# idcrook/tweeker_raytracer

Measured on NVIDIA B200. Metric: rtigo3_geometry_1080p_samples_per_s, higher is better.
Workload: dtype f32

## Files before the change

### tweeker_raytracer_b200/csrc/trace.cuh

```cuda
#pragma once

#include "rtc_internal.h"

#ifndef RTC_I2F_AXES
#define RTC_I2F_AXES 1
#endif
#ifndef RTC_RESTORE_WORLD
#define RTC_RESTORE_WORLD 1
#endif
#ifndef RTC_TRI_MINMAX
#define RTC_TRI_MINMAX 1
#endif
#ifndef RTC_LEAF_THRESHOLD
#define RTC_LEAF_THRESHOLD 0
#endif
#ifndef RTC_ONE_TRI_PER_STEP
#define RTC_ONE_TRI_PER_STEP 0
#endif
#ifndef RTC_FETCH_THRESHOLD
#define RTC_FETCH_THRESHOLD 12
#endif
#ifndef RTC_TRACE_MIN_BLOCKS
#define RTC_TRACE_MIN_BLOCKS 8
#endif

struct TraceHit
{
  float    t, u, v;
  uint32_t inst, prim;
};

struct ObjRay
{
  float dx, dy, dz;
  float Sx, Sy, Sz;
  int   kx, ky, kz;
};

__device__ __forceinline__ float sel3(float x, float y, float z, int k)
{
#if defined(__CUDACC__)
  float r;
  asm("{\n\t.reg .pred p1, p2;\n\tsetp.eq.s32 p1, %4, 1;\n\tsetp.eq.s32 p2, %4, 2;\n\tselp.f32 %0, %2, %1, p1;\n\tselp.f32 %0, %3, %0, p2;\n\t}"
      : "=&f"(r) : "f"(x), "f"(y), "f"(z), "r"(k));
  return r;
#else
  return (k == 2) ? z : ((k == 1) ? y : x);
#endif
}

__device__ __forceinline__ void shear_setup(ObjRay& r)
{
  const float ax = fabsf(r.dx), ay = fabsf(r.dy), az = fabsf(r.dz);
  int kz = (ax >= ay && ax >= az) ? 0 : ((ay >= az) ? 1 : 2);
  int kx = kz + 1; if (kx == 3) kx = 0;
  int ky = kx + 1; if (ky == 3) ky = 0;
  const float dz = sel3(r.dx, r.dy, r.dz, kz);
  if (dz < 0.0f) { const int t = kx; kx = ky; ky = t; }
  r.kx = kx; r.ky = ky; r.kz = kz;
  r.Sx = __fdiv_rn(sel3(r.dx, r.dy, r.dz, kx), dz);
  r.Sy = __fdiv_rn(sel3(r.dx, r.dy, r.dz, ky), dz);
  r.Sz = __fdiv_rn(1.0f, dz);
}

__device__ __forceinline__ float pick3(float x, float y, float z, bool is1, bool is2)
{
  float r = is1 ? y : x;
  return is2 ? z : r;
}

__device__ __forceinline__ bool tri_test(const ObjRay& r, float ox, float oy, float oz, const float4 v0, const float4 v1, const float4 v2,
                                         float& t, float& det, float& V, float& W)
{
  const float A0 = __fsub_rn(v0.x, ox), A1 = __fsub_rn(v0.y, oy), A2 = __fsub_rn(v0.z, oz);
  const float B0 = __fsub_rn(v1.x, ox), B1 = __fsub_rn(v1.y, oy), B2 = __fsub_rn(v1.z, oz);
  const float C0 = __fsub_rn(v2.x, ox), C1 = __fsub_rn(v2.y, oy), C2 = __fsub_rn(v2.z, oz);
  const bool x1 = r.kx == 1, x2 = r.kx == 2, y1 = r.ky == 1, y2 = r.ky == 2, z1 = r.kz == 1, z2 = r.kz == 2;
  const float Akz = pick3(A0, A1, A2, z1, z2), Bkz = pick3(B0, B1, B2, z1, z2), Ckz = pick3(C0, C1, C2, z1, z2);
  const float Ax = __fmaf_rn(-r.Sx, Akz, pick3(A0, A1, A2, x1, x2)), Ay = __fmaf_rn(-r.Sy, Akz, pick3(A0, A1, A2, y1, y2));
  const float Bx = __fmaf_rn(-r.Sx, Bkz, pick3(B0, B1, B2, x1, x2)), By = __fmaf_rn(-r.Sy, Bkz, pick3(B0, B1, B2, y1, y2));
  const float Cx = __fmaf_rn(-r.Sx, Ckz, pick3(C0, C1, C2, x1, x2)), Cy = __fmaf_rn(-r.Sy, Ckz, pick3(C0, C1, C2, y1, y2));
  float U = __fsub_rn(__fmul_rn(Cx, By), __fmul_rn(Cy, Bx));
  V = __fsub_rn(__fmul_rn(Ax, Cy), __fmul_rn(Ay, Cx));
  W = __fsub_rn(__fmul_rn(Bx, Ay), __fmul_rn(By, Ax));
  if (U == 0.0f || V == 0.0f || W == 0.0f)
  {
    U = (float)__dsub_rn(__dmul_rn((double)Cx, (double)By), __dmul_rn((double)Cy, (double)Bx));
    V = (float)__dsub_rn(__dmul_rn((double)Ax, (double)Cy), __dmul_rn((double)Ay, (double)Cx));
    W = (float)__dsub_rn(__dmul_rn((double)Bx, (double)Ay), __dmul_rn((double)By, (double)Ax));
  }
#if RTC_TRI_MINMAX
  if (fminf(fminf(U, V), W) < 0.0f && fmaxf(fmaxf(U, V), W) > 0.0f) return false;
#else
  if ((U < 0.0f || V < 0.0f || W < 0.0f) && (U > 0.0f || V > 0.0f || W > 0.0f)) return false;
#endif
  det = __fadd_rn(__fadd_rn(U, V), W);
  if (det == 0.0f) return false;
  const float Az = __fmul_rn(r.Sz, Akz), Bz = __fmul_rn(r.Sz, Bkz), Cz = __fmul_rn(r.Sz, Ckz);
  const float T = __fmaf_rn(U, Az, __fmaf_rn(V, Bz, __fmul_rn(W, Cz)));
  t = __fdiv_rn(T, det);
  return true;
}

struct BoxRay
{
  float idx, idy, idz;
  float ox, oy, oz;
  uint32_t octinv;
};

template <bool EXACT>
__device__ __forceinline__ float fast_rcp(float d)
{
  if (fabsf(d) < 0x1p-80f) d = copysignf(0x1p-80f, d);
  if (EXACT) return __frcp_rn(d);
#if defined(__CUDACC__)
  float r;
  asm("rcp.approx.ftz.f32 %0, %1;" : "=f"(r) : "f"(d));
  return r;
#else
  return 1.0f / d;
#endif
}

template <bool EXACT = false>
__device__ __forceinline__ void box_setup(BoxRay& b, float ox, float oy, float oz, float dx, float dy, float dz)
{
  b.idx = fast_rcp<EXACT>(dx); b.idy = fast_rcp<EXACT>(dy); b.idz = fast_rcp<EXACT>(dz);
  b.ox = ox; b.oy = oy; b.oz = oz;
  const uint32_t oct = ((dx < 0.0f) ? 4u : 0u) | ((dy < 0.0f) ? 2u : 0u) | ((dz < 0.0f) ? 1u : 0u);
  b.octinv = 7u ^ oct;
}

template <uint32_t I>
__device__ __forceinline__ float quant_f(uint32_t w, uint32_t bias)
{
#if defined(__CUDACC__)
  uint32_t r;
  asm("prmt.b32 %0, %1, %2, %3;" : "=r"(r) : "r"(w), "r"(bias), "n"(0x7404u | (I << 4)));
  return __uint_as_float(r);
#else
  return __uint_as_float((bias & 0xff000000u) | ((bias & 0xffu) << 16) | (((w >> (8u * I)) & 0xffu) << 8) | (bias & 0xffu));
#endif
}

template <uint32_t I>
__device__ __forceinline__ float quant_i2f(uint32_t w)
{
  return (float)((w >> (8u * I)) & 0xffu);
}

__device__ __forceinline__ float sat_idir(float id, uint32_t eb)
{
  const uint32_t raw = 0xB7000000u - (eb << 23);
  const float lim = __uint_as_float(raw < 0x7F000000u ? raw : 0x7F000000u);
  return fminf(fmaxf(id, -lim), lim);
}

__device__ __forceinline__ uint32_t node_test(const BoxRay& b, const uint4 n0, const uint4 n2, const uint4 n3, const uint4 n4,
                                              float tmin, float tlimit, uint32_t opaqueZero)
{
  const uint32_t e = n0.w;
  const float idx = sat_idir(b.idx, e & 0xffu), idy = sat_idir(b.idy, (e >> 8) & 0xffu), idz = sat_idir(b.idz, (e >> 16) & 0xffu);
  const float adjx = __uint_as_float((e & 0xffu) << 23) * idx;
  const float adjy = __uint_as_float(((e >> 8) & 0xffu) << 23) * idy;
  const float adjz = __uint_as_float(((e >> 16) & 0xffu) << 23) * idz;
  const float orgx = fmaf(-32768.0f, adjx, (__uint_as_float(n0.x) - b.ox) * idx);
#if RTC_I2F_AXES >= 2
  const float orgy = (__uint_as_float(n0.y) - b.oy) * idy;
#else
  const float orgy = fmaf(-32768.0f, adjy, (__uint_as_float(n0.y) - b.oy) * idy);
#endif
#if RTC_I2F_AXES >= 1
  const float orgz = (__uint_as_float(n0.z) - b.oz) * idz;
#else
  const float orgz = fmaf(-32768.0f, adjz, (__uint_as_float(n0.z) - b.oz) * idz);
#endif
  const bool nx = b.idx < 0.0f, ny = b.idy < 0.0f, nz = b.idz < 0.0f;
  const uint32_t nearx[2] = { nx ? n3.z : n2.x, nx ? n3.w : n2.y }, farx[2] = { nx ? n2.x : n3.z, nx ? n2.y : n3.w };
  const uint32_t neary[2] = { ny ? n4.x : n2.z, ny ? n4.y : n2.w }, fary[2] = { ny ? n2.z : n4.x, ny ? n2.w : n4.y };
  const uint32_t nearz[2] = { nz ? n4.z : n3.x, nz ? n4.w : n3.y }, farz[2] = { nz ? n3.x : n4.z, nz ? n3.y : n4.w };
  const float tlimitPad = tlimit * (1.0f + 0x1p-17f);
  const uint32_t bias = 0x47000000u + opaqueZero;
  uint32_t hits = 0;
#if RTC_I2F_AXES >= 1
#define RTC_QZ(I, W) quant_i2f<I>(W)
#else
#define RTC_QZ(I, W) quant_f<I>(W, bias)
#endif
#if RTC_I2F_AXES >= 2
#define RTC_QY(I, W) quant_i2f<I>(W)
#else
#define RTC_QY(I, W) quant_f<I>(W, bias)
#endif
#define RTC_BOX(S, H, I) \
  { \
    const float t0x = fmaf(quant_f<I>(nearx[H], bias), adjx, orgx), t1x = fmaf(quant_f<I>(farx[H], bias), adjx, orgx); \
    const float t0y = fmaf(RTC_QY(I, neary[H]), adjy, orgy), t1y = fmaf(RTC_QY(I, fary[H]), adjy, orgy); \
    const float t0z = fmaf(RTC_QZ(I, nearz[H]), adjz, orgz), t1z = fmaf(RTC_QZ(I, farz[H]), adjz, orgz); \
    const float tn = fmaxf(fmaxf(fmaxf(t0x, t0y), t0z), tmin); \
    const float tf = fminf(fminf(fminf(t1x, t1y), t1z) * (1.0f + 0x1p-17f), tlimitPad); \
    if (tn <= tf) hits |= 1u << S; \
  }
  RTC_BOX(0, 0, 0) RTC_BOX(1, 0, 1) RTC_BOX(2, 0, 2) RTC_BOX(3, 0, 3)
  RTC_BOX(4, 1, 0) RTC_BOX(5, 1, 1) RTC_BOX(6, 1, 2) RTC_BOX(7, 1, 3)
#undef RTC_BOX
#undef RTC_QZ
#undef RTC_QY
  return hits;
}

__device__ __forceinline__ uint32_t xor_permute8(uint32_t h, uint32_t x)
{
  if (x & 1u) h = ((h & 0xAAu) >> 1) | ((h & 0x55u) << 1);
  if (x & 2u) h = ((h & 0xCCu) >> 2) | ((h & 0x33u) << 2);
  if (x & 4u) h = ((h & 0xF0u) >> 4) | ((h & 0x0Fu) << 4);
  return h;
}

struct TraceCounts { uint32_t nodes, tris, insts; };

#define RTC_SM_STACK 8
#if RTC_RESTORE_WORLD
#define RTC_SM_RAY_WORDS 15
#else
#define RTC_SM_RAY_WORDS 11
#endif
#define RTC_LM_STACK 32

#ifndef RTC_STACK_OVERFLOW_COUNTER
#define RTC_STACK_OVERFLOW_COUNTER g_rtcStackOverflows
#endif
__device__ unsigned int RTC_STACK_OVERFLOW_COUNTER = 0;

template <bool ANY, bool COUNT, int BLOCK, bool SKIP = false, int TRICAP = RTC_ONE_TRI_PER_STEP>
struct Traversal
{
  float skipT; uint32_t skipInst, skipPrim;
  float* smRay;
  float tmin, tlimit;
  float hitT;
  uint32_t hitInst, hitPrim;
  uint2 nodeGroup, triGroup;
  int sp, blasBase;
  uint32_t curInst;
  BoxRay br;
  ObjRay orr;
  const uint4*  nodes;
  uint2* smStack;
  uint2* lmStack;
  TraceCounts counts;

  __device__ __forceinline__ void push(uint2 v)
  {
    if (sp < RTC_SM_STACK) smStack[sp * BLOCK] = v;
    else if (sp < RTC_SM_STACK + RTC_LM_STACK) lmStack[sp - RTC_SM_STACK] = v;
    else { atomicAdd(&RTC_STACK_OVERFLOW_COUNTER, 1u); return; }
    ++sp;
  }
  __device__ __forceinline__ uint2 pop()
  {
    --sp;
    return (sp < RTC_SM_STACK) ? smStack[sp * BLOCK] : lmStack[(sp - RTC_SM_STACK) & (RTC_LM_STACK - 1)];
  }

  __device__ __forceinline__ bool found() const { return hitInst != 0xffffffffu; }

  __device__ __forceinline__ TraceHit result() const
  {
    TraceHit h;
    h.t = -1.0f; h.u = 0.0f; h.v = 0.0f; h.inst = 0xffffffffu; h.prim = 0xffffffffu;
    if (found())
    {
      h.t = hitT; h.inst = hitInst; h.prim = hitPrim;
      if (!ANY) { const float det = smRay[8 * BLOCK]; h.u = __fdiv_rn(smRay[6 * BLOCK], det); h.v = __fdiv_rn(smRay[7 * BLOCK], det); }
    }
    return h;
  }

  __device__ __forceinline__ bool begin(const SceneDesc& sc, const float4 o, const float4 d)
  {
    smRay[0] = o.x; smRay[BLOCK] = o.y; smRay[2 * BLOCK] = o.z;
    smRay[3 * BLOCK] = d.x; smRay[4 * BLOCK] = d.y; smRay[5 * BLOCK] = d.z;
    tmin = o.w; tlimit = d.w;
    hitT = -1.0f; hitInst = 0xffffffffu; hitPrim = 0xffffffffu;
    if (COUNT) { counts.nodes = 0; counts.tris = 0; counts.insts = 0; }
    if (!(tlimit > tmin)) return false;
    sp = 0; blasBase = -1; curInst = 0;
    box_setup<COUNT>(br, o.x, o.y, o.z, d.x, d.y, d.z);
#if RTC_RESTORE_WORLD
    smRay[11 * BLOCK] = br.idx; smRay[12 * BLOCK] = br.idy; smRay[13 * BLOCK] = br.idz; smRay[14 * BLOCK] = __uint_as_float(br.octinv);
#endif
    nodes = sc.tlasNodes;
    nodeGroup = make_uint2(0u, 0x80000000u);
    triGroup = make_uint2(0u, 0u);
    return true;
  }

  __device__ __forceinline__ bool has_leaves() const { return triGroup.y != 0u; }

  __device__ __forceinline__ void node_phase()
  {
    if (nodeGroup.y & 0xff000000u)
    {
      const uint32_t bit = 31u - (uint32_t)__clz((int)nodeGroup.y);
      nodeGroup.y &= ~(1u << bit);
      if (nodeGroup.y & 0xff000000u) push(nodeGroup);
      const uint32_t slot = (bit - 24u) ^ br.octinv;
      const uint32_t rel = (uint32_t)__popc(nodeGroup.y & 0xffu & ((1u << slot) - 1u));
      const uint4* np = nodes + (size_t)(nodeGroup.x + rel) * 5u;
      const uint4 n0 = __ldg(np), n1 = __ldg(np + 1), n2 = __ldg(np + 2), n3 = __ldg(np + 3), n4 = __ldg(np + 4);
      if (COUNT) counts.nodes++;
      const uint32_t hits = node_test(br, n0, n2, n3, n4, tmin, tlimit, n1.x >> 31);
      const uint32_t imask = n0.w >> 24;
      nodeGroup = make_uint2(n1.x, (xor_permute8(hits & imask, br.octinv) << 24) | imask);
      uint32_t leaf = hits & ~imask, primMask = 0u;
      while (leaf)
      {
        const uint32_t s = (uint32_t)__ffs((int)leaf) - 1u;
        leaf &= leaf - 1u;
        const uint32_t meta = (((s < 4u) ? n1.z : n1.w) >> (8u * (s & 3u))) & 0xffu;
        primMask |= ((1u << (meta >> 5)) - 1u) << (meta & 31u);
      }
      triGroup = make_uint2(n1.y, primMask);
    }
    else
    {
      triGroup = nodeGroup;
      nodeGroup = make_uint2(0u, 0u);
    }
  }

  __device__ __forceinline__ bool leaf_phase(const SceneDesc& sc)
  {
    int tested = 0;
    while (triGroup.y)
    {
      const uint32_t idx = (uint32_t)__ffs((int)triGroup.y) - 1u;
      triGroup.y &= triGroup.y - 1u;
      if (blasBase < 0)
      {
        const uint32_t inst = __ldg(sc.tlasLeaves + triGroup.x + idx);
        if (triGroup.y) push(triGroup);
        if (nodeGroup.y & 0xff000000u) push(nodeGroup);
        const float4* ip = sc.instances + (size_t)inst * 4u;
        const float4 r0 = __ldg(ip), r1 = __ldg(ip + 1), r2 = __ldg(ip + 2), r3 = __ldg(ip + 3);
        if (COUNT) counts.insts++;
        const float wox = smRay[0], woy = smRay[BLOCK], woz = smRay[2 * BLOCK];
        const float wdx = smRay[3 * BLOCK], wdy = smRay[4 * BLOCK], wdz = smRay[5 * BLOCK];
        const float oox = __fmaf_rn(r0.x, wox, __fmaf_rn(r0.y, woy, __fmaf_rn(r0.z, woz, r0.w)));
        const float ooy = __fmaf_rn(r1.x, wox, __fmaf_rn(r1.y, woy, __fmaf_rn(r1.z, woz, r1.w)));
        const float ooz = __fmaf_rn(r2.x, wox, __fmaf_rn(r2.y, woy, __fmaf_rn(r2.z, woz, r2.w)));
        orr.dx = __fmaf_rn(r0.x, wdx, __fmaf_rn(r0.y, wdy, __fmul_rn(r0.z, wdz)));
        orr.dy = __fmaf_rn(r1.x, wdx, __fmaf_rn(r1.y, wdy, __fmul_rn(r1.z, wdz)));
        orr.dz = __fmaf_rn(r2.x, wdx, __fmaf_rn(r2.y, wdy, __fmul_rn(r2.z, wdz)));
        shear_setup(orr);
        box_setup<COUNT>(br, oox, ooy, ooz, orr.dx, orr.dy, orr.dz);
        curInst = inst;
        blasBase = sp;
        nodes = reinterpret_cast<const uint4*>(((unsigned long long)__float_as_uint(r3.y) << 32) | __float_as_uint(r3.x));
        smRay[9 * BLOCK] = r3.z; smRay[10 * BLOCK] = r3.w;
        nodeGroup = make_uint2(0u, 0x80000000u);
        triGroup = make_uint2(0u, 0u);
        break;
      }
      else
      {
        const float4* tris = reinterpret_cast<const float4*>(((unsigned long long)__float_as_uint(smRay[10 * BLOCK]) << 32) | __float_as_uint(smRay[9 * BLOCK]));
        const float4* tp = tris + (size_t)(triGroup.x + idx) * 3u;
        const float4 v0 = __ldg(tp), v1 = __ldg(tp + 1), v2 = __ldg(tp + 2);
        if (COUNT) counts.tris++;
        float t, det, V, W;
        if (tri_test(orr, br.ox, br.oy, br.oz, v0, v1, v2, t, det, V, W) && t > tmin)
        {
          const uint32_t prim = __float_as_uint(v0.w);
          if (SKIP && !(t > skipT || (t == skipT && (curInst > skipInst || (curInst == skipInst && prim > skipPrim))))) continue;
          if (ANY)
          {
            if (t < tlimit) { hitT = t; hitInst = curInst; hitPrim = prim; return false; }
          }
          else
          {
            const bool better = found() ? (t < hitT || (t == hitT && (curInst < hitInst || (curInst == hitInst && prim < hitPrim))))
                                      : (t < tlimit);
            if (better)
            {
              tlimit = t;
              hitT = t; hitInst = curInst; hitPrim = prim;
              smRay[6 * BLOCK] = V; smRay[7 * BLOCK] = W; smRay[8 * BLOCK] = det;
            }
          }
        }
        if (TRICAP == 1 || (TRICAP > 1 && ++tested >= TRICAP)) break;
      }
    }
    return true;
  }

  __device__ __forceinline__ bool advance(const SceneDesc& sc)
  {
    if (!(nodeGroup.y & 0xff000000u))
    {
      if (blasBase >= 0 && sp == blasBase)
      {
        blasBase = -1;
        nodes = sc.tlasNodes;
#if RTC_RESTORE_WORLD
        br.ox = smRay[0]; br.oy = smRay[BLOCK]; br.oz = smRay[2 * BLOCK];
        br.idx = smRay[11 * BLOCK]; br.idy = smRay[12 * BLOCK]; br.idz = smRay[13 * BLOCK]; br.octinv = __float_as_uint(smRay[14 * BLOCK]);
#else
        box_setup<COUNT>(br, smRay[0], smRay[BLOCK], smRay[2 * BLOCK], smRay[3 * BLOCK], smRay[4 * BLOCK], smRay[5 * BLOCK]);
#endif
      }
      if (sp == 0) return false;
      nodeGroup = pop();
    }
    return true;
  }

  __device__ __forceinline__ bool step(const SceneDesc& sc)
  {
    if (TRICAP > 0)
    {
      if (!(blasBase >= 0 && has_leaves())) node_phase();
      if (!leaf_phase(sc)) return false;
      if (blasBase >= 0 && has_leaves()) return true;
      return advance(sc);
    }
    node_phase();
    if (!leaf_phase(sc)) return false;
    return advance(sc);
  }
};

template <bool ANY, bool COUNT, int BLOCK, bool SKIP, int TRICAP = RTC_ONE_TRI_PER_STEP, class Policy>
__device__ __forceinline__ void trace_stream(const SceneDesc& sc, uint32_t n, uint32_t* __restrict__ cursor, Policy& policy, uint2* smem,
                                             unsigned long long* __restrict__ countsOut)
{
  Traversal<ANY, COUNT, BLOCK, SKIP, TRICAP> tr;
  uint2 overflow[RTC_LM_STACK];
  tr.smStack = smem + threadIdx.x;
  tr.smRay = reinterpret_cast<float*>(smem + RTC_SM_STACK * BLOCK) + threadIdx.x;
  tr.lmStack = overflow;
  const uint32_t lane = threadIdx.x & 31u;
  bool active = false, exhausted = false;
  uint32_t tag = 0;
  unsigned long long cNodes = 0, cTris = 0, cInsts = 0, cRays = 0;
  for (;;)
  {
    const uint32_t idle = __ballot_sync(0xffffffffu, !active);
    if (idle && !exhausted && (idle == 0xffffffffu || __popc(idle) >= RTC_FETCH_THRESHOLD))
    {
      const uint32_t want = (uint32_t)__popc(idle);
      const uint32_t leader = (uint32_t)__ffs((int)idle) - 1u;
      uint32_t base = 0;
      if (lane == leader) base = atomicAdd(cursor, want);
      base = __shfl_sync(0xffffffffu, base, leader);
      if (base + want >= n) exhausted = true;
      if (!active)
      {
        const uint32_t index = base + (uint32_t)__popc(idle & ((1u << lane) - 1u));
        if (index < n)
        {
          float4 o, d;
          if (policy.load(index, o, d, tag))
          {
            if constexpr (SKIP) policy.skip_key(tag, tr.skipT, tr.skipInst, tr.skipPrim);
            if (tr.begin(sc, o, d)) active = true;
            else { policy.store(tag, tr.result()); if (COUNT) cRays++; }
          }
        }
      }
    }
    else if (idle == 0xffffffffu) break;
#if RTC_LEAF_THRESHOLD > 0
    bool running = active;
    if (active && !tr.has_leaves()) tr.node_phase();
    const bool held = active && tr.has_leaves();
    const uint32_t heldLanes = __ballot_sync(0xffffffffu, held), activeLanes = ~idle;
    if (heldLanes)
    {
      const uint32_t nHeld = (uint32_t)__popc(heldLanes), nActive = (uint32_t)__popc(activeLanes);
      if (nHeld >= RTC_LEAF_THRESHOLD || nHeld * 4u >= nActive)
      {
        if (held) running = tr.leaf_phase(sc);
      }
    }
    if (running && !tr.has_leaves()) running = tr.advance(sc);
    if (active && !running)
    {
      policy.store(tag, tr.result());
      if (COUNT) { cNodes += tr.counts.nodes; cTris += tr.counts.tris; cInsts += tr.counts.insts; cRays++; }
      active = false;
    }
#else
    if (active)
    {
      if (!tr.step(sc))
      {
        policy.store(tag, tr.result());
        if (COUNT) { cNodes += tr.counts.nodes; cTris += tr.counts.tris; cInsts += tr.counts.insts; cRays++; }
        active = false;
      }
    }
#endif
  }
  if (COUNT)
  {
    for (int off = 16; off; off >>= 1)
    {
      cNodes += __shfl_down_sync(0xffffffffu, cNodes, off); cTris += __shfl_down_sync(0xffffffffu, cTris, off);
      cInsts += __shfl_down_sync(0xffffffffu, cInsts, off); cRays += __shfl_down_sync(0xffffffffu, cRays, off);
    }
    if (lane == 0 && cRays)
    {
      atomicAdd(countsOut + 0, cNodes); atomicAdd(countsOut + 1, cTris); atomicAdd(countsOut + 2, cInsts); atomicAdd(countsOut + 3, cRays);
    }
  }
}
```

Baseline: 2618.

## Add warp-cooperative triangle pass and enable int-to-float decode on Y axis

Switches the default RTC_I2F_AXES to 2, so Y-axis box-plane dequantization uses plain int-to-float conversion (node_test becomes templated on the axis count). Packs the shear axis indices into one word, merges hitT into tlimit, and factors instance entry and hit acceptance into helpers. Adds an optional warp-cooperative triangle pass that spreads pending triangles across lanes and reduces the closest hit through a shared table, disabled by default via RTC_WARP_PASS=0. The I2F change trims ALU work per node test, and the struct slimming may reduce register pressure.

```diff
diff --git a/tweeker_raytracer_b200/csrc/trace.cuh b/tweeker_raytracer_b200/csrc/trace.cuh
--- a/tweeker_raytracer_b200/csrc/trace.cuh
+++ b/tweeker_raytracer_b200/csrc/trace.cuh
@@ -3,7 +3,7 @@
 #include "rtc_internal.h"
 
 #ifndef RTC_I2F_AXES
-#define RTC_I2F_AXES 1
+#define RTC_I2F_AXES 2
 #endif
 #ifndef RTC_RESTORE_WORLD
 #define RTC_RESTORE_WORLD 1
@@ -19,6 +19,9 @@
 #endif
 #ifndef RTC_FETCH_THRESHOLD
 #define RTC_FETCH_THRESHOLD 12
+#endif
+#ifndef RTC_WARP_PASS
+#define RTC_WARP_PASS 0
 #endif
 #ifndef RTC_TRACE_MIN_BLOCKS
 #define RTC_TRACE_MIN_BLOCKS 8
@@ -34,7 +37,7 @@
 {
   float dx, dy, dz;
   float Sx, Sy, Sz;
-  int   kx, ky, kz;
+  uint32_t k;
 };
 
 __device__ __forceinline__ float sel3(float x, float y, float z, int k)
@@ -57,7 +60,7 @@
   int ky = kx + 1; if (ky == 3) ky = 0;
   const float dz = sel3(r.dx, r.dy, r.dz, kz);
   if (dz < 0.0f) { const int t = kx; kx = ky; ky = t; }
-  r.kx = kx; r.ky = ky; r.kz = kz;
+  r.k = (uint32_t)kx | ((uint32_t)ky << 2) | ((uint32_t)kz << 4);
   r.Sx = __fdiv_rn(sel3(r.dx, r.dy, r.dz, kx), dz);
   r.Sy = __fdiv_rn(sel3(r.dx, r.dy, r.dz, ky), dz);
   r.Sz = __fdiv_rn(1.0f, dz);
@@ -75,7 +78,7 @@
   const float A0 = __fsub_rn(v0.x, ox), A1 = __fsub_rn(v0.y, oy), A2 = __fsub_rn(v0.z, oz);
   const float B0 = __fsub_rn(v1.x, ox), B1 = __fsub_rn(v1.y, oy), B2 = __fsub_rn(v1.z, oz);
   const float C0 = __fsub_rn(v2.x, ox), C1 = __fsub_rn(v2.y, oy), C2 = __fsub_rn(v2.z, oz);
-  const bool x1 = r.kx == 1, x2 = r.kx == 2, y1 = r.ky == 1, y2 = r.ky == 2, z1 = r.kz == 1, z2 = r.kz == 2;
+  const bool x1 = (r.k & 1u) != 0u, x2 = (r.k & 2u) != 0u, y1 = (r.k & 4u) != 0u, y2 = (r.k & 8u) != 0u, z1 = (r.k & 16u) != 0u, z2 = (r.k & 32u) != 0u;
   const float Akz = pick3(A0, A1, A2, z1, z2), Bkz = pick3(B0, B1, B2, z1, z2), Ckz = pick3(C0, C1, C2, z1, z2);
   const float Ax = __fmaf_rn(-r.Sx, Akz, pick3(A0, A1, A2, x1, x2)), Ay = __fmaf_rn(-r.Sy, Akz, pick3(A0, A1, A2, y1, y2));
   const float Bx = __fmaf_rn(-r.Sx, Bkz, pick3(B0, B1, B2, x1, x2)), By = __fmaf_rn(-r.Sy, Bkz, pick3(B0, B1, B2, y1, y2));
@@ -157,6 +160,7 @@
   return fminf(fmaxf(id, -lim), lim);
 }
 
+template <int AXES>
 __device__ __forceinline__ uint32_t node_test(const BoxRay& b, const uint4 n0, const uint4 n2, const uint4 n3, const uint4 n4,
                                               float tmin, float tlimit, uint32_t opaqueZero)
 {
@@ -166,16 +170,8 @@
   const float adjy = __uint_as_float(((e >> 8) & 0xffu) << 23) * idy;
   const float adjz = __uint_as_float(((e >> 16) & 0xffu) << 23) * idz;
   const float orgx = fmaf(-32768.0f, adjx, (__uint_as_float(n0.x) - b.ox) * idx);
-#if RTC_I2F_AXES >= 2
-  const float orgy = (__uint_as_float(n0.y) - b.oy) * idy;
-#else
-  const float orgy = fmaf(-32768.0f, adjy, (__uint_as_float(n0.y) - b.oy) * idy);
-#endif
-#if RTC_I2F_AXES >= 1
-  const float orgz = (__uint_as_float(n0.z) - b.oz) * idz;
-#else
-  const float orgz = fmaf(-32768.0f, adjz, (__uint_as_float(n0.z) - b.oz) * idz);
-#endif
+  const float orgy = AXES >= 2 ? (__uint_as_float(n0.y) - b.oy) * idy : fmaf(-32768.0f, adjy, (__uint_as_float(n0.y) - b.oy) * idy);
+  const float orgz = AXES >= 1 ? (__uint_as_float(n0.z) - b.oz) * idz : fmaf(-32768.0f, adjz, (__uint_as_float(n0.z) - b.oz) * idz);
   const bool nx = b.idx < 0.0f, ny = b.idy < 0.0f, nz = b.idz < 0.0f;
   const uint32_t nearx[2] = { nx ? n3.z : n2.x, nx ? n3.w : n2.y }, farx[2] = { nx ? n2.x : n3.z, nx ? n2.y : n3.w };
   const uint32_t neary[2] = { ny ? n4.x : n2.z, ny ? n4.y : n2.w }, fary[2] = { ny ? n2.z : n4.x, ny ? n2.w : n4.y };
@@ -183,16 +179,8 @@
   const float tlimitPad = tlimit * (1.0f + 0x1p-17f);
   const uint32_t bias = 0x47000000u + opaqueZero;
   uint32_t hits = 0;
-#if RTC_I2F_AXES >= 1
-#define RTC_QZ(I, W) quant_i2f<I>(W)
-#else
-#define RTC_QZ(I, W) quant_f<I>(W, bias)
-#endif
-#if RTC_I2F_AXES >= 2
-#define RTC_QY(I, W) quant_i2f<I>(W)
-#else
-#define RTC_QY(I, W) quant_f<I>(W, bias)
-#endif
+#define RTC_QZ(I, W) (AXES >= 1 ? quant_i2f<I>(W) : quant_f<I>(W, bias))
+#define RTC_QY(I, W) (AXES >= 2 ? quant_i2f<I>(W) : quant_f<I>(W, bias))
 #define RTC_BOX(S, H, I) \
   { \
     const float t0x = fmaf(quant_f<I>(nearx[H], bias), adjx, orgx), t1x = fmaf(quant_f<I>(farx[H], bias), adjx, orgx); \
@@ -239,7 +227,6 @@
   float skipT; uint32_t skipInst, skipPrim;
   float* smRay;
   float tmin, tlimit;
-  float hitT;
   uint32_t hitInst, hitPrim;
   uint2 nodeGroup, triGroup;
   int sp, blasBase;
@@ -272,7 +259,7 @@
     h.t = -1.0f; h.u = 0.0f; h.v = 0.0f; h.inst = 0xffffffffu; h.prim = 0xffffffffu;
     if (found())
     {
-      h.t = hitT; h.inst = hitInst; h.prim = hitPrim;
+      h.t = tlimit; h.inst = hitInst; h.prim = hitPrim;
       if (!ANY) { const float det = smRay[8 * BLOCK]; h.u = __fdiv_rn(smRay[6 * BLOCK], det); h.v = __fdiv_rn(smRay[7 * BLOCK], det); }
     }
     return h;
@@ -283,7 +270,7 @@
     smRay[0] = o.x; smRay[BLOCK] = o.y; smRay[2 * BLOCK] = o.z;
     smRay[3 * BLOCK] = d.x; smRay[4 * BLOCK] = d.y; smRay[5 * BLOCK] = d.z;
     tmin = o.w; tlimit = d.w;
-    hitT = -1.0f; hitInst = 0xffffffffu; hitPrim = 0xffffffffu;
+    hitInst = 0xffffffffu; hitPrim = 0xffffffffu;
     if (COUNT) { counts.nodes = 0; counts.tris = 0; counts.insts = 0; }
     if (!(tlimit > tmin)) return false;
     sp = 0; blasBase = -1; curInst = 0;
@@ -311,7 +298,7 @@
       const uint4* np = nodes + (size_t)(nodeGroup.x + rel) * 5u;
       const uint4 n0 = __ldg(np), n1 = __ldg(np + 1), n2 = __ldg(np + 2), n3 = __ldg(np + 3), n4 = __ldg(np + 4);
       if (COUNT) counts.nodes++;
-      const uint32_t hits = node_test(br, n0, n2, n3, n4, tmin, tlimit, n1.x >> 31);
+      const uint32_t hits = node_test<COUNT ? 1 : RTC_I2F_AXES>(br, n0, n2, n3, n4, tmin, tlimit, n1.x >> 31);
       const uint32_t imask = n0.w >> 24;
       nodeGroup = make_uint2(n1.x, (xor_permute8(hits & imask, br.octinv) << 24) | imask);
       uint32_t leaf = hits & ~imask, primMask = 0u;
@@ -331,6 +318,53 @@
     }
   }
 
+  static __device__ __forceinline__ const float4* tri_array(const float* column)
+  {
+    return reinterpret_cast<const float4*>(((unsigned long long)__float_as_uint(column[10 * BLOCK]) << 32) | __float_as_uint(column[9 * BLOCK]));
+  }
+
+  __device__ __forceinline__ uint32_t pass_word(int k) const
+  {
+    switch (k)
+    {
+      case 0: return __float_as_uint(br.ox);
+      case 1: return __float_as_uint(br.oy);
+      case 2: return __float_as_uint(br.oz);
+      case 3: return __float_as_uint(orr.Sx);
+      case 4: return __float_as_uint(orr.Sy);
+      case 5: return __float_as_uint(orr.Sz);
+      case 6: return orr.k;
+      case 7: return __float_as_uint(tmin);
+      default: return triGroup.x;
+    }
+  }
+
+  __device__ __forceinline__ void enter_instance(const SceneDesc& sc, uint32_t idx)
+  {
+    const uint32_t inst = __ldg(sc.tlasLeaves + triGroup.x + idx);
+    if (triGroup.y) push(triGroup);
+    if (nodeGroup.y & 0xff000000u) push(nodeGroup);
+    const float4* ip = sc.instances + (size_t)inst * 4u;
+    const float4 r0 = __ldg(ip), r1 = __ldg(ip + 1), r2 = __ldg(ip + 2), r3 = __ldg(ip + 3);
+    if (COUNT) counts.insts++;
+    const float wox = smRay[0], woy = smRay[BLOCK], woz = smRay[2 * BLOCK];
+    const float wdx = smRay[3 * BLOCK], wdy = smRay[4 * BLOCK], wdz = smRay[5 * BLOCK];
+    const float oox = __fmaf_rn(r0.x, wox, __fmaf_rn(r0.y, woy, __fmaf_rn(r0.z, woz, r0.w)));
+    const float ooy = __fmaf_rn(r1.x, wox, __fmaf_rn(r1.y, woy, __fmaf_rn(r1.z, woz, r1.w)));
+    const float ooz = __fmaf_rn(r2.x, wox, __fmaf_rn(r2.y, woy, __fmaf_rn(r2.z, woz, r2.w)));
+    orr.dx = __fmaf_rn(r0.x, wdx, __fmaf_rn(r0.y, wdy, __fmul_rn(r0.z, wdz)));
+    orr.dy = __fmaf_rn(r1.x, wdx, __fmaf_rn(r1.y, wdy, __fmul_rn(r1.z, wdz)));
+    orr.dz = __fmaf_rn(r2.x, wdx, __fmaf_rn(r2.y, wdy, __fmul_rn(r2.z, wdz)));
+    shear_setup(orr);
+    box_setup<COUNT>(br, oox, ooy, ooz, orr.dx, orr.dy, orr.dz);
+    curInst = inst;
+    blasBase = sp;
+    nodes = reinterpret_cast<const uint4*>(((unsigned long long)__float_as_uint(r3.y) << 32) | __float_as_uint(r3.x));
+    smRay[9 * BLOCK] = r3.z; smRay[10 * BLOCK] = r3.w;
+    nodeGroup = make_uint2(0u, 0x80000000u);
+    triGroup = make_uint2(0u, 0u);
+  }
+
   __device__ __forceinline__ bool leaf_phase(const SceneDesc& sc)
   {
     int tested = 0;
@@ -340,34 +374,12 @@
       triGroup.y &= triGroup.y - 1u;
       if (blasBase < 0)
       {
-        const uint32_t inst = __ldg(sc.tlasLeaves + triGroup.x + idx);
-        if (triGroup.y) push(triGroup);
-        if (nodeGroup.y & 0xff000000u) push(nodeGroup);
-        const float4* ip = sc.instances + (size_t)inst * 4u;
-        const float4 r0 = __ldg(ip), r1 = __ldg(ip + 1), r2 = __ldg(ip + 2), r3 = __ldg(ip + 3);
-        if (COUNT) counts.insts++;
-        const float wox = smRay[0], woy = smRay[BLOCK], woz = smRay[2 * BLOCK];
-        const float wdx = smRay[3 * BLOCK], wdy = smRay[4 * BLOCK], wdz = smRay[5 * BLOCK];
-        const float oox = __fmaf_rn(r0.x, wox, __fmaf_rn(r0.y, woy, __fmaf_rn(r0.z, woz, r0.w)));
-        const float ooy = __fmaf_rn(r1.x, wox, __fmaf_rn(r1.y, woy, __fmaf_rn(r1.z, woz, r1.w)));
-        const float ooz = __fmaf_rn(r2.x, wox, __fmaf_rn(r2.y, woy, __fmaf_rn(r2.z, woz, r2.w)));
-        orr.dx = __fmaf_rn(r0.x, wdx, __fmaf_rn(r0.y, wdy, __fmul_rn(r0.z, wdz)));
-        orr.dy = __fmaf_rn(r1.x, wdx, __fmaf_rn(r1.y, wdy, __fmul_rn(r1.z, wdz)));
-        orr.dz = __fmaf_rn(r2.x, wdx, __fmaf_rn(r2.y, wdy, __fmul_rn(r2.z, wdz)));
-        shear_setup(orr);
-        box_setup<COUNT>(br, oox, ooy, ooz, orr.dx, orr.dy, orr.dz);
-        curInst = inst;
-        blasBase = sp;
-        nodes = reinterpret_cast<const uint4*>(((unsigned long long)__float_as_uint(r3.y) << 32) | __float_as_uint(r3.x));
-        smRay[9 * BLOCK] = r3.z; smRay[10 * BLOCK] = r3.w;
-        nodeGroup = make_uint2(0u, 0x80000000u);
-        triGroup = make_uint2(0u, 0u);
+        enter_instance(sc, idx);
         break;
       }
       else
       {
-        const float4* tris = reinterpret_cast<const float4*>(((unsigned long long)__float_as_uint(smRay[10 * BLOCK]) << 32) | __float_as_uint(smRay[9 * BLOCK]));
-        const float4* tp = tris + (size_t)(triGroup.x + idx) * 3u;
+        const float4* tp = tri_array(smRay) + (size_t)(triGroup.x + idx) * 3u;
         const float4 v0 = __ldg(tp), v1 = __ldg(tp + 1), v2 = __ldg(tp + 2);
         if (COUNT) counts.tris++;
         float t, det, V, W;
@@ -375,24 +387,27 @@
         {
           const uint32_t prim = __float_as_uint(v0.w);
           if (SKIP && !(t > skipT || (t == skipT && (curInst > skipInst || (curInst == skipInst && prim > skipPrim))))) continue;
-          if (ANY)
-          {
-            if (t < tlimit) { hitT = t; hitInst = curInst; hitPrim = prim; return false; }
-          }
-          else
-          {
-            const bool better = found() ? (t < hitT || (t == hitT && (curInst < hitInst || (curInst == hitInst && prim < hitPrim))))
-                                      : (t < tlimit);
-            if (better)
-            {
-              tlimit = t;
-              hitT = t; hitInst = curInst; hitPrim = prim;
-              smRay[6 * BLOCK] = V; smRay[7 * BLOCK] = W; smRay[8 * BLOCK] = det;
-            }
-          }
+          if (!accept(t, prim, V, W, det)) return false;
         }
         if (TRICAP == 1 || (TRICAP > 1 && ++tested >= TRICAP)) break;
       }
+    }
+    return true;
+  }
+
+  __device__ __forceinline__ bool accept(float t, uint32_t prim, float V, float W, float det)
+  {
+    if (ANY)
+    {
+      if (t < tlimit) { tlimit = t; hitInst = curInst; hitPrim = prim; return false; }
+      return true;
+    }
+    const bool better = found() ? (t < tlimit || (t == tlimit && (curInst < hitInst || (curInst == hitInst && prim < hitPrim))))
+                              : (t < tlimit);
+    if (better)
+    {
+      tlimit = t; hitInst = curInst; hitPrim = prim;
+      smRay[6 * BLOCK] = V; smRay[7 * BLOCK] = W; smRay[8 * BLOCK] = det;
     }
     return true;
   }
@@ -433,6 +448,142 @@
   }
 };
 
+struct PassLane
+{
+  bool running;
+  uint32_t cnt;
+  uint32_t range;
+  uint32_t entry;
+  uint32_t ray[9];
+  unsigned long long key;
+  float t, V, W, det;
+};
+
+__device__ __forceinline__ uint32_t* key_word(unsigned long long* tab, uint32_t l, int h) { return reinterpret_cast<uint32_t*>(tab + l) + h; }
+
+template <class Wp>
+__device__ __forceinline__ void tri_pass(Wp& w)
+{
+  w.each([](uint32_t, auto& tr, PassLane& s) { s.cnt = (s.running && tr.blasBase >= 0) ? (uint32_t)__popc(tr.triGroup.y) : 0u; });
+  if (!w.ballot([](uint32_t, auto&, PassLane& s) { return s.cnt != 0u; })) return;
+  w.scan([](uint32_t, auto&, PassLane& s) { return s.cnt; },
+         [](uint32_t, auto&, PassLane& s, uint32_t sum) {
+           s.range = (s.cnt != 0u && sum <= 32u) ? (uint32_t)(((1ull << s.cnt) - 1ull) << (sum - s.cnt)) : 0u;
+           s.cnt = sum;
+         });
+  const uint32_t fit = w.ballot([](uint32_t, auto&, PassLane& s) { return s.cnt <= 32u; });
+  uint32_t used = 0;
+  w.shfl([](uint32_t, auto&, PassLane& s) { return s.cnt; }, [fit](uint32_t, auto&, PassLane&) { return 31u - (uint32_t)__clz((int)fit); },
+         [&used](uint32_t, auto&, PassLane&, uint32_t v) { used = v; });
+  unsigned long long* tab = w.table();
+  w.sync();
+  w.each([&w, tab](uint32_t l, auto& tr, PassLane& s) {
+    if (!s.range) return;
+    w.posted(l, tr.triGroup.y);
+    uint32_t slot = (uint32_t)__ffs((int)s.range) - 1u;
+    for (uint32_t m = tr.triGroup.y; m; m &= m - 1u) tab[slot++] = (l << 5) | ((uint32_t)__ffs((int)m) - 1u);
+    tr.triGroup.y = 0u;
+  });
+  w.sync();
+  w.each([used, tab](uint32_t l, auto&, PassLane& s) { s.entry = l < used ? (uint32_t)tab[l] : ~0u; });
+#pragma unroll
+  for (int k = 0; k < 9; ++k)
+    w.shfl([k](uint32_t, auto& tr, PassLane&) { return tr.pass_word(k); }, [](uint32_t, auto&, PassLane& s) { return s.entry >> 5; },
+           [k](uint32_t, auto&, PassLane& s, uint32_t v) { s.ray[k] = v; });
+  w.sync();
+  w.each([tab](uint32_t l, auto&, PassLane& s) { if (s.range) tab[l] = ~0ull; });
+  w.sync();
+  w.each([&w, tab](uint32_t l, auto& tr, PassLane& s) {
+    s.key = ~0ull;
+    if (s.entry == ~0u) return;
+    const uint32_t owner = s.entry >> 5, idx = s.entry & 31u;
+    w.tested(owner, idx);
+    const float4* tp = tr.tri_array(w.column(tr, l, owner)) + (size_t)(s.ray[8] + idx) * 3u;
+    const float4 v0 = __ldg(tp), v1 = __ldg(tp + 1), v2 = __ldg(tp + 2);
+    ObjRay r;
+    r.Sx = __uint_as_float(s.ray[3]); r.Sy = __uint_as_float(s.ray[4]); r.Sz = __uint_as_float(s.ray[5]);
+    r.k = s.ray[6];
+    float t, det, V, W;
+    if (tri_test(r, __uint_as_float(s.ray[0]), __uint_as_float(s.ray[1]), __uint_as_float(s.ray[2]), v0, v1, v2, t, det, V, W)
+        && t > __uint_as_float(s.ray[7]))
+    {
+      const uint32_t u = __float_as_uint(__fadd_rn(t, 0.0f));
+      s.key = ((unsigned long long)(u ^ ((uint32_t)((int32_t)u >> 31) | 0x80000000u)) << 32) | __float_as_uint(v0.w);
+      s.t = t; s.V = V; s.W = W; s.det = det;
+      w.atomic_min(key_word(tab, owner, 1), (uint32_t)(s.key >> 32));
+    }
+  });
+  w.sync();
+  w.each([&w, tab](uint32_t, auto&, PassLane& s) {
+    if (s.key != ~0ull && *key_word(tab, s.entry >> 5, 1) == (uint32_t)(s.key >> 32)) w.atomic_min(key_word(tab, s.entry >> 5, 0), (uint32_t)s.key);
+  });
+  w.sync();
+  const uint32_t win = w.ballot([tab](uint32_t, auto&, PassLane& s) { return s.key != ~0ull && tab[s.entry >> 5] == s.key; });
+  w.each([win](uint32_t l, auto&, PassLane& s) { const uint32_t mine = s.range & win; s.entry = mine ? (uint32_t)__ffs((int)mine) - 1u : l; });
+  w.shfl([](uint32_t, auto&, PassLane& s) { return __float_as_uint(s.t); }, [](uint32_t, auto&, PassLane& s) { return s.entry; },
+         [](uint32_t, auto&, PassLane& s, uint32_t v) { s.t = __uint_as_float(v); });
+  w.shfl([](uint32_t, auto&, PassLane& s) { return __float_as_uint(s.V); }, [](uint32_t, auto&, PassLane& s) { return s.entry; },
+         [](uint32_t, auto&, PassLane& s, uint32_t v) { s.V = __uint_as_float(v); });
+  w.shfl([](uint32_t, auto&, PassLane& s) { return __float_as_uint(s.W); }, [](uint32_t, auto&, PassLane& s) { return s.entry; },
+         [](uint32_t, auto&, PassLane& s, uint32_t v) { s.W = __uint_as_float(v); });
+  w.shfl([](uint32_t, auto&, PassLane& s) { return __float_as_uint(s.det); }, [](uint32_t, auto&, PassLane& s) { return s.entry; },
+         [](uint32_t, auto&, PassLane& s, uint32_t v) { s.det = __uint_as_float(v); });
+  w.each([win, tab](uint32_t l, auto& tr, PassLane& s) {
+    if (s.range & win) s.running = tr.accept(s.t, (uint32_t)tab[l], s.V, s.W, s.det);
+  });
+}
+
+template <class Wp>
+__device__ __forceinline__ void warp_step(Wp& w, const SceneDesc& sc)
+{
+  w.each([&sc](uint32_t, auto& tr, PassLane& s) {
+    if (!s.running) return;
+    if (!(tr.blasBase >= 0 && tr.has_leaves())) tr.node_phase();
+    if (tr.blasBase < 0 && tr.has_leaves())
+    {
+      const uint32_t idx = (uint32_t)__ffs((int)tr.triGroup.y) - 1u;
+      tr.triGroup.y &= tr.triGroup.y - 1u;
+      tr.enter_instance(sc, idx);
+    }
+  });
+  tri_pass(w);
+  w.each([&sc](uint32_t, auto& tr, PassLane& s) {
+    if (s.running && !(tr.blasBase >= 0 && tr.has_leaves())) s.running = tr.advance(sc);
+  });
+}
+
+#if defined(__CUDACC__)
+template <class Tr>
+struct WarpLane
+{
+  Tr& tr; PassLane& s; uint32_t lane; unsigned long long* tab;
+
+  template <class F> __device__ __forceinline__ void each(F f) { f(lane, tr, s); }
+  template <class F> __device__ __forceinline__ uint32_t ballot(F p) { return __ballot_sync(0xffffffffu, p(lane, tr, s)); }
+  template <class G, class S, class P> __device__ __forceinline__ void shfl(G get, S src, P put)
+  {
+    put(lane, tr, s, __shfl_sync(0xffffffffu, get(lane, tr, s), src(lane, tr, s)));
+  }
+  template <class G, class P> __device__ __forceinline__ void scan(G get, P put)
+  {
+    uint32_t v = get(lane, tr, s);
+#pragma unroll
+    for (uint32_t d = 1; d < 32u; d <<= 1)
+    {
+      const uint32_t u = __shfl_up_sync(0xffffffffu, v, d);
+      if (lane >= d) v += u;
+    }
+    put(lane, tr, s, v);
+  }
+  __device__ __forceinline__ void sync() { __syncwarp(); }
+  __device__ __forceinline__ unsigned long long* table() { return tab; }
+  __device__ __forceinline__ void atomic_min(uint32_t* p, uint32_t v) { atomicMin(p, v); }
+  __device__ __forceinline__ const float* column(const Tr& t, uint32_t l, uint32_t owner) const { return t.smRay + ((int)owner - (int)l); }
+  __device__ __forceinline__ void posted(uint32_t, uint32_t) {}
+  __device__ __forceinline__ void tested(uint32_t, uint32_t) {}
+};
+#endif
+
 template <bool ANY, bool COUNT, int BLOCK, bool SKIP, int TRICAP = RTC_ONE_TRI_PER_STEP, class Policy>
 __device__ __forceinline__ void trace_stream(const SceneDesc& sc, uint32_t n, uint32_t* __restrict__ cursor, Policy& policy, uint2* smem,
                                              unsigned long long* __restrict__ countsOut)
@@ -443,6 +594,9 @@
   tr.smRay = reinterpret_cast<float*>(smem + RTC_SM_STACK * BLOCK) + threadIdx.x;
   tr.lmStack = overflow;
   const uint32_t lane = threadIdx.x & 31u;
+#if defined(__CUDACC__)
+  constexpr bool kWarpPass = RTC_WARP_PASS && !COUNT && !SKIP && TRICAP == 0;
+#endif
   bool active = false, exhausted = false;
   uint32_t tag = 0;
   unsigned long long cNodes = 0, cTris = 0, cInsts = 0, cRays = 0;
@@ -494,6 +648,22 @@
       active = false;
     }
 #else
+#if defined(__CUDACC__)
+    if constexpr (kWarpPass)
+    {
+      __shared__ unsigned long long passTable[BLOCK];
+      PassLane s;
+      s.running = active;
+      WarpLane<decltype(tr)> w{ tr, s, lane, passTable + (threadIdx.x & ~31u) };
+      warp_step(w, sc);
+      if (active && !s.running)
+      {
+        policy.store(tag, tr.result());
+        active = false;
+      }
+    }
+    else
+#endif
     if (active)
     {
       if (!tr.step(sc))
```

New measurement: 2647 (median of 6 runs). 1.1% higher.
